# zhengyk19/vit-rpe-rope

Measured on AMD Instinct MI355X. Metric: train images/sec, CIFAR-10 ViT d=192 L=6 H=6, higher is better.
Workload: dtype bf16; 1 GPU; CIFAR-10-shaped 32x32 patch4 ViT d=192 L=6 H=6, --pos_encoding rope-axial theta=100, bf16, full train step (fwd+CE+bwd+AdamW), random-init weights; per_gpu_batch=512, global_batch=512, parallelism=dp1, hip_graph=True

## Files before the change

vit-rpe-rope_amd/csrc/tail2.hip:

```cpp
#include "common.h"
#include <type_traits>
#include <stdlib.h>

#ifndef T2_RB
#define T2_RB 6
#endif
#ifndef T2_NV
#define T2_NV 8
#endif

namespace vitpe {

struct Tail2Args {
  const void* a;
  const void* xin;
  const void* wp;
  const float* bp;
  const float* gamma;
  const float* beta;
  const void* w1;
  const float* b1;
  const void* w2;
  const float* b2;
  void* xmid;
  float* mean2;
  float* rstd2;
  void* xn_out;
  void* gp_out;
  void* h_out;
  void* out;
  float* mean_out;
  float* rstd_out;
  int M, HID;
  float eps2, eps_next;
  unsigned long long* census;
};

constexpr int T2_D = 192, T2_NT = 12, T2_KS = 6, T2_WAVES = 9;
constexpr int T2_THREADS = 64 * (T2_WAVES + 2);
constexpr int T2F_THREADS = 64 * (T2_WAVES + 3);
constexpr int T2_MAXHID = 1536, T2_NFLAG = T2_MAXHID / 64 + 10;
constexpr int T2_CH = 64, T2_CNT = T2_CH / 16, T2_CKS = T2_CH / 32;
constexpr int T2_HALF = T2_CNT * T2_KS;
constexpr int T2_SLABF = 2 * T2_HALF;
static_assert(T2_NT * T2_CKS == T2_HALF, "slab halves");

VITPE_DEV float t2_xg_sum(float v) {
  auto r = __builtin_amdgcn_permlane16_swap(__float_as_uint(v), __float_as_uint(v), false, false);
  v = __uint_as_float(r[0]) + __uint_as_float(r[1]);
  auto q = __builtin_amdgcn_permlane32_swap(__float_as_uint(v), __float_as_uint(v), false, false);
  return __uint_as_float(q[0]) + __uint_as_float(q[1]);
}

#ifndef T2_LOADER_PRIO
#define T2_LOADER_PRIO 3
#endif
#ifndef T2_AUX_HID
#define T2_AUX_HID 2
#endif
#ifndef T2_AUX_ROW
#define T2_AUX_ROW 0
#endif
struct T2Row {
  __amdgpu_buffer_rsrc_t rsrc;
  int off;
  VITPE_DEV T2Row operator+(int elems) const { return T2Row{rsrc, off + 2 * elems}; }
};
VITPE_DEV T2Row t2_row(void* base, int row0, int row, int ld) {
  const __amdgpu_buffer_rsrc_t r = __builtin_amdgcn_make_buffer_rsrc(reinterpret_cast<bf16*>(base) + (size_t)row0 * ld, 0, 0x7fffffff, 0x00020000);
  return T2Row{r, (row - row0) * ld * 2};
}
typedef __attribute__((ext_vector_type(4))) unsigned t2_u32x4;

template <int AUX>
VITPE_DEV void t2_store_pair(const T2Row& row, int nt0, int g, const f32x4& o0, const f32x4& o1) {
  uint32_t lo[2], hi[2];
#pragma unroll
  for (int w2 = 0; w2 < 2; ++w2) {
    bf16x2 pa, pb;
    pa[0] = (bf16)o0[2 * w2]; pa[1] = (bf16)o0[2 * w2 + 1];
    pb[0] = (bf16)o1[2 * w2]; pb[1] = (bf16)o1[2 * w2 + 1];
    const auto r = __builtin_amdgcn_permlane16_swap(__builtin_bit_cast(uint32_t, pa), __builtin_bit_cast(uint32_t, pb), false, false);
    lo[w2] = r[0]; hi[w2] = r[1];
  }
  const int f0 = 16 * (nt0 + (g & 1)) + 8 * (g >> 1);
  __builtin_amdgcn_raw_buffer_store_b128((t2_u32x4){lo[0], lo[1], hi[0], hi[1]}, row.rsrc, row.off + 2 * f0, 0, AUX);
}

template <int AUX>
VITPE_DEV void t2_store_pair_f16(const T2Row& row, int nt0, int g, const f32x4& o0, const f32x4& o1) {
  uint32_t lo[2], hi[2];
#pragma unroll
  for (int w2 = 0; w2 < 2; ++w2) {
    const uint32_t pa = __builtin_bit_cast(uint32_t, __builtin_amdgcn_cvt_pkrtz(o0[2 * w2], o0[2 * w2 + 1]));
    const uint32_t pb = __builtin_bit_cast(uint32_t, __builtin_amdgcn_cvt_pkrtz(o1[2 * w2], o1[2 * w2 + 1]));
    const auto r = __builtin_amdgcn_permlane16_swap(pa, pb, false, false);
    lo[w2] = r[0]; hi[w2] = r[1];
  }
  const int f0 = 16 * (nt0 + (g & 1)) + 8 * (g >> 1);
  __builtin_amdgcn_raw_buffer_store_b128((t2_u32x4){lo[0], lo[1], hi[0], hi[1]}, row.rsrc, row.off + 2 * f0, 0, AUX);
}

template <int AUX>
VITPE_DEV void t2_store_frag(const T2Row& row, int ks, int g, const Frag<bf16>& f) {
  const t2_u32x4 d = __builtin_bit_cast(t2_u32x4, f.v);
  const auto r0 = __builtin_amdgcn_permlane16_swap(d[0], d[2], false, false);
  const auto r1 = __builtin_amdgcn_permlane16_swap(d[1], d[3], false, false);
  const int f0 = 16 * (2 * ks + (g & 1)) + 8 * (g >> 1);
  __builtin_amdgcn_raw_buffer_store_b128((t2_u32x4){r0[0], r1[0], r0[1], r1[1]}, row.rsrc, row.off + 2 * f0, 0, AUX);
}

template <int NTL, int KSL, int R>
VITPE_DEV void t2_gemm_code(const bf16* wb, const Frag<bf16>* bf, f32x4* acc) {
  constexpr int TOT = NTL * KSL;
  static_assert(TOT >= R, "ring deeper than the product");
  Frag<bf16> w[R];
#pragma unroll
  for (int i = 0; i < R - 1; ++i) w[i] = ld_frag(wb + ((i % NTL) * KSL + i / NTL) * 512);
#pragma unroll
  for (int q = 0; q < TOT; ++q) {
    if (q + R - 1 < TOT) {
      const int n = q + R - 1;
      w[n % R] = ld_frag(wb + ((n % NTL) * KSL + n / NTL) * 512);
    }
    mma(w[q % R], bf[q / NTL], acc[q % NTL]);
  }
}
template <int TOT, int R, int NV>
VITPE_DEV void t2_gemm_order() {
  __builtin_amdgcn_sched_group_barrier(0x100, R - 1, 0);
#pragma unroll
  for (int q = 0; q < TOT; ++q) {
    if (q + R - 1 < TOT) __builtin_amdgcn_sched_group_barrier(0x100, 1, 0);
    __builtin_amdgcn_sched_group_barrier(0x008, 1, 0);
    if (NV > 0) __builtin_amdgcn_sched_group_barrier(0x002, NV, 0);
  }
}
template <int NTL, int KSL, int R>
VITPE_DEV void t2_gemm(const bf16* wb, const Frag<bf16>* bf, f32x4* acc) {
  __builtin_amdgcn_sched_barrier(0);
  t2_gemm_code<NTL, KSL, R>(wb, bf, acc);
  t2_gemm_order<NTL * KSL, R, 0>();
  __builtin_amdgcn_sched_barrier(0);
}

VITPE_DEV void t2_gelu(float x, float& h, float& g) {
  constexpr float C = 0.39894228040143267794f;
  const float ax = fabsf(x);
  const float T = __builtin_amdgcn_rcpf(fmaf(ax, 0.3275911f * 0.70710678118654752440f, 1.0f));
  float q = fmaf(T, 1.061405429f / (2.f * C), -1.453152027f / (2.f * C));
  q = fmaf(T, q, 1.421413741f / (2.f * C));
  q = fmaf(T, q, -0.284496736f / (2.f * C));
  q = fmaf(T, q, 0.254829592f / (2.f * C));
  const float E = __builtin_amdgcn_exp2f(fmaf(x * x, -0.72134752044448170368f, -1.32574806473615827f));
  const float H = (q * T) * E;
  h = fmaf(-ax, H, fmaxf(x, 0.f));
  const float r = fmaf(ax, E, -H);
  g = x >= 0.f ? 1.0f + r : -r;
}

template <bool F1, bool F2, int NV, int R = 8, class GFn>
VITPE_DEV void t2_step(const bf16* w1f, const bf16* w2f, const Frag<bf16> (&bf)[T2_KS], f32x4 (&a1n)[2],
                       const Frag<bf16>& hprev, f32x4 (&acc2)[T2_NT], GFn gfn) {
  constexpr int TOT = (F1 ? 12 : 0) + (F2 ? 12 : 0);
  __builtin_amdgcn_sched_barrier(0);
  if (TOT > 0) {
    auto frag_ptr = [&](int q) -> const bf16* {
      const bool is2 = (F1 && F2) ? (q % 2 == 0) : F2;
      const int j = (F1 && F2) ? q / 2 : q;
// ... 307 lines not shown
      }
    }
    stamp(8);

    {
      const T2Row outr = t2_row(a.out, 16 * tile0, rowc, D);
      float s1 = 0.f;
  #pragma unroll
      for (int nt = 0; nt < NT; ++nt) {
        const f32x4 rv = ld4(xmr + 16 * nt + 4 * g);
  #pragma unroll
        for (int r = 0; r < 4; ++r) { acc2[nt][r] = to_f32(from_f32<T>(acc2[nt][r] + rv[r])); s1 += acc2[nt][r]; }
      }
  #pragma unroll
      for (int nt = 0; nt < NT; nt += 2) t2_store_pair<T2_AUX_ROW>(outr, nt, g, acc2[nt], acc2[nt + 1]);
      if (a.mean_out != nullptr) {
        const float mean = t2_xg_sum(s1) * invD;
        float s2 = 0.f;
  #pragma unroll
        for (int nt = 0; nt < NT; ++nt)
  #pragma unroll
          for (int r = 0; r < 4; ++r) { const float d = acc2[nt][r] - mean; s2 += d * d; }
        const float var = t2_xg_sum(s2) * invD;
        if (g == 0) { a.mean_out[rowc] = mean; a.rstd_out[rowc] = 1.0f / sqrtf(var + a.eps_next); }
      }
    }
    stamp(9);
  };
  if (half >= 0) body(std::true_type{});
  else body(std::false_type{});
}

struct Tail2BwdArgs {
  const void* dy;
  const void* gp;
  const void* xmid;
  const float* mean2;
  const float* rstd2;
  const float* gamma;
  const void* w2t;
  const void* w1t;
  const void* wpt;
  void* du;
  void* dxmid;
  void* da;
  float* dgamma;
  float* dbeta;
  int M, HID;
  const void* dqkv;
  const void* wqt;
  const void* x1;
  const float* mean1;
  const float* rstd1;
  const float* gamma1;
  const void* dres1;
  float* dgamma1;
  float* dbeta1;
  int K1;
};

VITPE_DEV void t2_unpack_pair(const Chunk16& v, f32x4& o0, f32x4& o1) {
#pragma unroll
  for (int w2 = 0; w2 < 2; ++w2) {
    const auto r = __builtin_amdgcn_permlane16_swap(v[w2], v[2 + w2], false, false);
    o0[2 * w2] = __uint_as_float(r[0] << 16);
    o0[2 * w2 + 1] = __uint_as_float(r[0] & 0xffff0000u);
    o1[2 * w2] = __uint_as_float(r[1] << 16);
    o1[2 * w2 + 1] = __uint_as_float(r[1] & 0xffff0000u);
  }
}

VITPE_DEV void t2_unpack_pair_f16(const Chunk16& v, f32x4& o0, f32x4& o1) {
#pragma unroll
  for (int w2 = 0; w2 < 2; ++w2) {
    const auto r = __builtin_amdgcn_permlane16_swap(v[w2], v[2 + w2], false, false);
    const uint32_t ra = r[0], rb = r[1];
    o0[2 * w2] = (float)__builtin_bit_cast(_Float16, (unsigned short)(ra & 0xffffu));
    o0[2 * w2 + 1] = (float)__builtin_bit_cast(_Float16, (unsigned short)(ra >> 16));
    o1[2 * w2] = (float)__builtin_bit_cast(_Float16, (unsigned short)(rb & 0xffffu));
    o1[2 * w2 + 1] = (float)__builtin_bit_cast(_Float16, (unsigned short)(rb >> 16));
  }
}

template <int CTRL> VITPE_DEV float t2_dppc(float v) {
  return __builtin_bit_cast(float, __builtin_amdgcn_update_dpp(0, __builtin_bit_cast(int, v), CTRL, 0xf, 0xf, true));
}
VITPE_DEV float t2_colsum8(const float (&t)[8], int c) {
  const bool b3 = (c & 8) != 0, b2 = (c & 4) != 0, b1 = (c & 2) != 0;
  float u[4], w[2];
#pragma unroll
  for (int k = 0; k < 4; ++k) u[k] = (b3 ? t[4 + k] : t[k]) + t2_dppc<0x128>(b3 ? t[k] : t[4 + k]);
#pragma unroll
  for (int k = 0; k < 2; ++k) w[k] = (b2 ? u[2 + k] : u[k]) + t2_dppc<0x141>(b2 ? u[k] : u[2 + k]);
  const float x = (b1 ? w[1] : w[0]) + t2_dppc<0x4E>(b1 ? w[0] : w[1]);
  return x + t2_dppc<0xB1>(x);
}

VITPE_DEV void t2_ln_backward(f32x4 (&acc)[T2_NT], const bf16* xrow, const bf16* rrow, float mean, float rstd,
                              const float* sGam, float* sAcc, int c, int g, float valid, const T2Row& orow) {
  constexpr int D = T2_D, NT = T2_NT;
  bf16x4 xmv[NT];
#pragma unroll
  for (int nt = 0; nt < NT; ++nt) xmv[nt] = *reinterpret_cast<const bf16x4*>(xrow + 16 * nt);
  const float invD = 1.0f / (float)D;
  float s1 = 0.f, s2 = 0.f;
#pragma unroll
  for (int nt = 0; nt < NT; ++nt) {
    __builtin_amdgcn_sched_barrier(0);
    const f32x4 gam = *reinterpret_cast<const f32x4*>(sGam + 16 * nt + 4 * g);
    float tot[8];
#pragma unroll
    for (int r = 0; r < 4; ++r) {
      const float xhat = ((float)xmv[nt][r] - mean) * rstd;
      const float dxn = acc[nt][r];
      tot[r] = dxn * xhat * valid;
      tot[4 + r] = dxn * valid;
      const float gy = dxn * gam[r];
      s1 += gy;
      s2 = fmaf(gy, xhat, s2);
    }
    const float sel = t2_colsum8(tot, c);
    asm volatile("" : "+v"(s1), "+v"(s2));
    if (!(c & 1)) atomicAdd(&sAcc[(c < 8 ? 0 : D - 4) + 16 * nt + 4 * g + (c >> 1)], sel);
  }
  const float m1 = t2_xg_sum(s1) * invD, m2 = t2_xg_sum(s2) * invD;
  bf16x4 rv[NT];
#pragma unroll
  for (int nt = 0; nt < NT; ++nt) rv[nt] = *reinterpret_cast<const bf16x4*>(rrow + 16 * nt);
#pragma unroll
  for (int nt = 0; nt < NT; ++nt) {
    __builtin_amdgcn_sched_barrier(0);
    uint2 xw = __builtin_bit_cast(uint2, xmv[nt]);
    asm volatile("" : "+v"(xw.x), "+v"(xw.y));
    const bf16x4 xb = __builtin_bit_cast(bf16x4, xw);
    const f32x4 gam = *reinterpret_cast<const f32x4*>(sGam + 16 * nt + 4 * g);
#pragma unroll
    for (int r = 0; r < 4; ++r) {
      const float xhat = ((float)xb[r] - mean) * rstd;
      const float gy = acc[nt][r] * gam[r];
      acc[nt][r] = to_f32(from_f32<bf16>(fmaf(rstd, gy - m1 - xhat * m2, (float)rv[nt][r])));
    }
  }
#pragma unroll
  for (int nt = 0; nt < NT; nt += 2) t2_store_pair<T2_AUX_ROW>(orow, nt, g, acc[nt], acc[nt + 1]);
}

VITPE_DEV void t2_flush_colsums(float* sAcc, int* sFin, int nactive, int lane, float* dgamma, float* dbeta) {
  asm volatile("s_waitcnt lgkmcnt(0)" ::: "memory");
  int fin = 0;
  if (lane == 0) fin = atomicAdd(sFin, 1);
  fin = __builtin_amdgcn_readfirstlane(fin);
  if (fin == nactive - 1) {
    for (int i = lane; i < T2_D; i += 64) {
      atomicAdd(dgamma + i, __hip_atomic_load(&sAcc[i], __ATOMIC_RELAXED, __HIP_MEMORY_SCOPE_WORKGROUP));
      atomicAdd(dbeta + i, __hip_atomic_load(&sAcc[T2_D + i], __ATOMIC_RELAXED, __HIP_MEMORY_SCOPE_WORKGROUP));
    }
  }
}

template <bool PRE>
__global__ __launch_bounds__(T2_THREADS) void block_tail2_bwd_kernel(Tail2BwdArgs a) {
  using T = bf16;
  constexpr int D = T2_D, NT = T2_NT, KS = T2_KS;
  __shared__ __attribute__((aligned(16))) T sW[3 * T2_SLABF * 512];
  __shared__ __attribute__((aligned(16))) float sGam[T2_D], sGam1[PRE ? T2_D : 4];
  __shared__ float sAcc[2 * T2_D], sAcc1[PRE ? 2 * T2_D : 4];
  __shared__ int sReady[T2_NFLAG], sDone[T2_NFLAG], sFin;

  const int lane = threadIdx.x & 63, c = lane & 15, g = lane >> 4;
  const int wave = __builtin_amdgcn_readfirstlane(threadIdx.x >> 6);
  const int HID = a.HID, nchunk = HID / T2_CH, nsub = 2 * nchunk;
  const int nkc = PRE ? a.K1 / 64 : 0, Q = (nkc + 1) / 2, QB = nkc / 2;
  const int ntiles = (a.M + 15) / 16, base = ntiles / (int)gridDim.x, rem = ntiles % (int)gridDim.x;
  const int tile0 = (int)blockIdx.x * base + min((int)blockIdx.x, rem), ntile_wg = base + ((int)blockIdx.x < rem ? 1 : 0);
  const bool active = wave < ntile_wg;
  const int row = 16 * (tile0 + wave) + c;
  const int rowc = min(row, a.M - 1);
  const float valid = row < a.M ? 1.0f : 0.0f;

  if (threadIdx.x < T2_NFLAG) { sReady[threadIdx.x] = 0; sDone[threadIdx.x] = 0; }
  if (threadIdx.x == 0) sFin = 0;
  for (int i = threadIdx.x; i < 2 * D; i += T2_THREADS) { sAcc[i] = 0.f; if (PRE) sAcc1[i] = 0.f; }
  for (int i = threadIdx.x; i < D; i += T2_THREADS) { sGam[i] = a.gamma[i]; if (PRE) sGam1[i] = a.gamma1[i]; }

  auto dma1 = [&](const T* src_frag, int dst_frag) {
    __builtin_amdgcn_global_load_lds((const __attribute__((address_space(1))) void*)(src_frag + lane * 8),
                                     (__attribute__((address_space(3))) void*)(sW + dst_frag * 512), 16, 0, 0);
  };
  if (wave >= T2_WAVES) {
    __builtin_amdgcn_s_setprio(T2_LOADER_PRIO);
    const bool is1 = wave == T2_WAVES;
    const int nq = is1 ? Q : QB, njobs = nq + nchunk;
    const int half = is1 ? 0 : T2_HALF;
    auto job_slab = [&](int j) { return j < nq ? j : Q + (j - nq) + (is1 ? 0 : 1); };
    auto dma_job = [&](int j) {
      const T* src;
      if (j < nq) src = reinterpret_cast<const T*>(a.wqt) + ((size_t)j * T2_SLABF + half) * 512;
      else src = (is1 ? reinterpret_cast<const T*>(a.w2t) : reinterpret_cast<const T*>(a.w1t)) + (size_t)(j - nq) * T2_HALF * 512;
      const int b0 = ((job_slab(j) + 2) % 3) * T2_SLABF + half;
#pragma unroll
      for (int f = 0; f < T2_HALF; ++f) dma1(src + (size_t)f * 512, b0 + f);
    };
    auto wait_done = [&](int k) {
      while (__builtin_amdgcn_readfirstlane(__hip_atomic_load(&sDone[k], __ATOMIC_RELAXED, __HIP_MEMORY_SCOPE_WORKGROUP)) < ntile_wg)
        __builtin_amdgcn_s_sleep(2);
      asm volatile("" ::: "memory");
    };
    auto raise = [&](int sl) {
      asm volatile("" ::: "memory");
      if (lane == 0) atomicAdd(&sReady[sl], 1);
    };
    __builtin_amdgcn_s_waitcnt(0x0070);
    asm volatile("s_barrier" ::: "memory");
    int issued = 0, raised = 0;
    auto top_up = [&]() {
      while (issued < njobs && issued - raised < 2) {
        const int g2 = job_slab(issued);
        if (g2 >= 3) {
          if (raised < issued && job_slab(raised) <= g2 - 3) break;
          wait_done(g2 - 2);
        }
        dma_job(issued++);
      }
    };
    top_up();
    while (raised < njobs) {
      if (issued - raised - 1 >= 1) __builtin_amdgcn_s_waitcnt(0x4F78);
      else __builtin_amdgcn_s_waitcnt(0x0F70);
      raise(job_slab(raised));
      ++raised;
      top_up();
    }
    wait_done(Q + nchunk + 1);
#pragma unroll
    for (int f = 0; f < NT * KS / 2; ++f) {
      const int ff = (is1 ? 0 : NT * KS / 2) + f;
      dma1(reinterpret_cast<const T*>(a.wpt) + (size_t)ff * 512, ff);
    }
    __builtin_amdgcn_s_waitcnt(0x0F70);
    raise(Q + nchunk + 1);
    return;
  }
  auto wait_ready = [&](int gs) {
    const int s = gs - Q;
    const int need = gs < Q ? 1 + (2 * gs + 1 < nkc ? 1 : 0) : s > nchunk ? 2 : (s < nchunk ? 1 : 0) + (s >= 1 ? 1 : 0);
    while (__builtin_amdgcn_readfirstlane(__hip_atomic_load(&sReady[gs], __ATOMIC_RELAXED, __HIP_MEMORY_SCOPE_WORKGROUP)) < need)
      __builtin_amdgcn_s_sleep(1);
    asm volatile("" ::: "memory");
  };
  auto signal_done = [&](int k) {
    asm volatile("s_waitcnt lgkmcnt(0)" ::: "memory");
    if (lane == 0) atomicAdd(&sDone[k], 1);
  };
  auto slab_ptr = [&](int gs) { return sW + ((gs + 2) % 3) * T2_SLABF * 512 + lane * 8; };

  Frag<T> bf[KS];
  const T* const dqr = PRE ? reinterpret_cast<const T*>(a.dqkv) + (size_t)rowc * a.K1 + 8 * g : nullptr;
  Frag<T> bqa[4], bqb[4];
  if (active) {
    if (PRE) {
#pragma unroll
      for (int i = 0; i < 4; ++i) bqa[i] = ld_frag(dqr + 32 * min(i, a.K1 / 32 - 1));
    } else {
      const T* dr = reinterpret_cast<const T*>(a.dy) + (size_t)rowc * D + 4 * g;
#pragma unroll
      for (int ks = 0; ks < KS; ++ks) {
        const bf16x4 lo = *reinterpret_cast<const bf16x4*>(dr + 32 * ks), hi = *reinterpret_cast<const bf16x4*>(dr + 32 * ks + 16);
        bf[ks].v = __builtin_shufflevector(lo, hi, 0, 1, 2, 3, 4, 5, 6, 7);
      }
    }
  }
  __builtin_amdgcn_s_waitcnt(0x0070);
  asm volatile("s_barrier" ::: "memory");
  if (!active) return;

  if (PRE) {
    f32x4 acc[NT];
#pragma unroll
    for (int nt = 0; nt < NT; ++nt) acc[nt] = (f32x4){0.f, 0.f, 0.f, 0.f};
    const int nks = a.K1 / 32;
    auto qslab = [&](int q, const Frag<T> (&cur)[4], Frag<T> (&nxt)[4]) {
      if (q + 1 < Q) {
#pragma unroll
        for (int i = 0; i < 4; ++i) nxt[i] = ld_frag(dqr + 32 * min(4 * (q + 1) + i, nks - 1));
      }
      wait_ready(q);
      const T* wb = slab_ptr(q);
      t2_gemm<NT, 2, 8>(wb, cur, acc);
      if (4 * q + 2 < nks) t2_gemm<NT, 2, 8>(wb + T2_HALF * 512, cur + 2, acc);
      signal_done(q + 1);
    };
    for (int q = 0; q < Q; q += 2) {
      qslab(q, bqa, bqb);
      if (q + 1 < Q) qslab(q + 1, bqb, bqa);
    }
    t2_ln_backward(acc, reinterpret_cast<const T*>(a.x1) + (size_t)rowc * D + 4 * g,
                   reinterpret_cast<const T*>(a.dres1) + (size_t)rowc * D + 4 * g, a.mean1[rowc], a.rstd1[rowc], sGam1, sAcc1,
                   c, g, valid, t2_row(const_cast<void*>(a.dy), 16 * tile0, rowc, D));
#pragma unroll
    for (int ks = 0; ks < KS; ++ks) bf[ks] = acc_to_frag<T>(acc[2 * ks], acc[2 * ks + 1]);
  }

  const T* const gpr = reinterpret_cast<const T*>(a.gp) + (size_t)rowc * HID + 16 * (g & 1) + 8 * (g >> 1);
  const T2Row dur = t2_row(a.du, 16 * tile0, rowc, HID);
  Chunk16 gq[2];
#pragma unroll
  for (int t = 0; t < 2; ++t) gq[t] = *reinterpret_cast<const Chunk16*>(gpr + 32 * t);
  f32x4 acc2[NT];
#pragma unroll
  for (int nt = 0; nt < NT; ++nt) acc2[nt] = (f32x4){0.f, 0.f, 0.f, 0.f};
  f32x4 aX[2], aY[2];
  Frag<T> hP, hQ;
  const f32x4 z4 = {0.f, 0.f, 0.f, 0.f};
  auto gstage = [&](const f32x4 (&a1c)[2], Chunk16& slot, int t, Frag<T>& hnew) {
    f32x4 g0, g1, d0, d1;
    t2_unpack_pair_f16(slot, g0, g1);
    if (t + 2 < nsub) slot = *reinterpret_cast<const Chunk16*>(gpr + 32 * (t + 2));
#pragma unroll
    for (int r = 0; r < 4; ++r) { d0[r] = a1c[0][r] * g0[r]; d1[r] = a1c[1][r] * g1[r]; }
    t2_store_pair<T2_AUX_HID>(dur + 32 * t, 0, g, d0, d1);
    hnew = acc_to_frag<T>(d0, d1);
  };
  constexpr int NVB = 3, RB = T2_RB;

  wait_ready(Q);
  {
    const T* wb = slab_ptr(Q);
    aX[0] = z4; aX[1] = z4;
    t2_step<true, false, 0, RB>(wb, wb, bf, aX, hQ, acc2, [&]() {});
    aY[0] = z4; aY[1] = z4;
    t2_step<true, false, 2 * NVB, RB>(wb + 2 * KS * 512, wb, bf, aY, hQ, acc2, [&]() { gstage(aX, gq[0], 0, hP); });
    signal_done(Q + 1);
  }
  for (int p = 1; p < nchunk; ++p) {
    wait_ready(Q + p);
    const T* wb = slab_ptr(Q + p);
    const T* w2b = wb + T2_HALF * 512;
    aX[0] = z4; aX[1] = z4;
    t2_step<true, true, NVB, RB>(wb, w2b, bf, aX, hP, acc2, [&]() { gstage(aY, gq[1], 2 * p - 1, hQ); });
    aY[0] = z4; aY[1] = z4;
    t2_step<true, true, NVB, RB>(wb + 2 * KS * 512, w2b + NT * 512, bf, aY, hQ, acc2, [&]() { gstage(aX, gq[0], 2 * p, hP); });
    signal_done(Q + p + 1);
  }
  wait_ready(Q + nchunk);
  {
    const T* w2b = slab_ptr(Q + nchunk) + T2_HALF * 512;
    const int tl = nsub - 1;
    t2_step<false, true, 2 * NVB, RB>(w2b, w2b, bf, aX, hP, acc2, [&]() { gstage(aY, gq[1], tl, hQ); });
    t2_step<false, true, 0, RB>(w2b, w2b + NT * 512, bf, aX, hQ, acc2, [&]() {});
    signal_done(Q + nchunk + 1);
  }
  t2_ln_backward(acc2, reinterpret_cast<const T*>(a.xmid) + (size_t)rowc * D + 4 * g,
                 reinterpret_cast<const T*>(a.dy) + (size_t)rowc * D + 4 * g, a.mean2[rowc], a.rstd2[rowc], sGam, sAcc, c, g,
                 valid, t2_row(a.dxmid, 16 * tile0, rowc, D));
#pragma unroll
  for (int ks = 0; ks < KS; ++ks) bf[ks] = acc_to_frag<T>(acc2[2 * ks], acc2[2 * ks + 1]);
  f32x4 accA[NT];
#pragma unroll
  for (int nt = 0; nt < NT; ++nt) accA[nt] = z4;
  wait_ready(Q + nchunk + 1);
  t2_gemm<NT, KS, 12>(sW + lane * 8, bf, accA);
  {
    const T2Row dar = t2_row(a.da, 16 * tile0, rowc, D);
#pragma unroll
    for (int nt = 0; nt < NT; nt += 2) t2_store_pair<T2_AUX_ROW>(dar, nt, g, accA[nt], accA[nt + 1]);
  }
  asm volatile("s_waitcnt lgkmcnt(0)" ::: "memory");
  int fin = 0;
  if (lane == 0) fin = atomicAdd(&sFin, 1);
  fin = __builtin_amdgcn_readfirstlane(fin);
  if (fin == ntile_wg - 1) {
    for (int i = lane; i < D; i += 64) {
      atomicAdd(a.dgamma + i, __hip_atomic_load(&sAcc[i], __ATOMIC_RELAXED, __HIP_MEMORY_SCOPE_WORKGROUP));
      atomicAdd(a.dbeta + i, __hip_atomic_load(&sAcc[D + i], __ATOMIC_RELAXED, __HIP_MEMORY_SCOPE_WORKGROUP));
      if (PRE) {
        atomicAdd(a.dgamma1 + i, __hip_atomic_load(&sAcc1[i], __ATOMIC_RELAXED, __HIP_MEMORY_SCOPE_WORKGROUP));
        atomicAdd(a.dbeta1 + i, __hip_atomic_load(&sAcc1[D + i], __ATOMIC_RELAXED, __HIP_MEMORY_SCOPE_WORKGROUP));
      }
    }
  }
}

struct LnBwd2Args {
  const void* dy;
  const void* wt;
  const void* x;
  const float* mean;
  const float* rstd;
  const float* gamma;
  const void* dres;
  void* dx;
  float* dgamma;
  float* dbeta;
  int M, K;
};

__global__ __launch_bounds__(T2_THREADS) void ln_bwd2_kernel(LnBwd2Args a) {
  using T = bf16;
  constexpr int D = T2_D, NT = T2_NT, KS = T2_KS, SLF = NT * KS;
  __shared__ __attribute__((aligned(16))) T sW[2 * SLF * 512];
  __shared__ __attribute__((aligned(16))) float sGam[T2_D];
  __shared__ float sAcc[2 * T2_D];
  __shared__ int sReady[T2_NFLAG], sDone[T2_NFLAG], sFin;

  const int lane = threadIdx.x & 63, c = lane & 15, g = lane >> 4;
  const int wave = __builtin_amdgcn_readfirstlane(threadIdx.x >> 6);
  const int K = a.K, nslab = K / D;
  const int ntiles = (a.M + 15) / 16, base = ntiles / (int)gridDim.x, rem = ntiles % (int)gridDim.x;
  const int tile0 = (int)blockIdx.x * base + min((int)blockIdx.x, rem), ntile_wg = base + ((int)blockIdx.x < rem ? 1 : 0);
  const bool active = wave < ntile_wg;
  const int row = 16 * (tile0 + wave) + c;
  const int rowc = min(row, a.M - 1);
  const float valid = row < a.M ? 1.0f : 0.0f;

  if (threadIdx.x < T2_NFLAG) { sReady[threadIdx.x] = 0; sDone[threadIdx.x] = 0; }
  if (threadIdx.x == 0) sFin = 0;
  for (int i = threadIdx.x; i < 2 * D; i += T2_THREADS) sAcc[i] = 0.f;
  for (int i = threadIdx.x; i < D; i += T2_THREADS) sGam[i] = a.gamma[i];

  if (wave >= T2_WAVES) {
    __builtin_amdgcn_s_setprio(T2_LOADER_PRIO);
    const int half = wave == T2_WAVES ? 0 : SLF / 2;
    auto dma_half = [&](int sl) {
#pragma unroll
      for (int f = 0; f < SLF / 2; ++f) {
        const T* src = reinterpret_cast<const T*>(a.wt) + ((size_t)sl * SLF + half + f) * 512 + lane * 8;
        __builtin_amdgcn_global_load_lds((const __attribute__((address_space(1))) void*)src,
                                         (__attribute__((address_space(3))) void*)(sW + ((sl & 1) * SLF + half + f) * 512), 16, 0, 0);
      }
    };
    __builtin_amdgcn_s_waitcnt(0x0070);
    asm volatile("s_barrier" ::: "memory");
    dma_half(0);
    if (nslab > 1) dma_half(1);
    for (int sl = 0; sl < nslab; ++sl) {
      if (sl + 1 < nslab) asm volatile("s_waitcnt vmcnt(36)" ::: "memory");
      else __builtin_amdgcn_s_waitcnt(0x0F70);
      asm volatile("" ::: "memory");
      if (lane == 0) atomicAdd(&sReady[sl], 1);
      if (sl + 2 < nslab) {
        while (__builtin_amdgcn_readfirstlane(__hip_atomic_load(&sDone[sl], __ATOMIC_RELAXED, __HIP_MEMORY_SCOPE_WORKGROUP)) < ntile_wg)
          __builtin_amdgcn_s_sleep(2);
        asm volatile("" ::: "memory");
        dma_half(sl + 2);
      }
    }
    return;
  }
  __builtin_amdgcn_s_waitcnt(0x0070);
  asm volatile("s_barrier" ::: "memory");
  if (!active) return;

  const T* const dr = reinterpret_cast<const T*>(a.dy) + (size_t)rowc * K + 8 * g;
  Frag<T> bfa[KS], bfb[KS];
#pragma unroll
  for (int ks = 0; ks < KS; ++ks) bfa[ks] = ld_frag(dr + 32 * ks);
  f32x4 acc[NT];
#pragma unroll
  for (int nt = 0; nt < NT; ++nt) acc[nt] = (f32x4){0.f, 0.f, 0.f, 0.f};
  auto chunk = [&](int sl, const Frag<T> (&cur)[KS], Frag<T> (&nxt)[KS]) {
    if (sl + 1 < nslab) {
#pragma unroll
      for (int ks = 0; ks < KS; ++ks) nxt[ks] = ld_frag(dr + (sl + 1) * D + 32 * ks);
    }
    while (__builtin_amdgcn_readfirstlane(__hip_atomic_load(&sReady[sl], __ATOMIC_RELAXED, __HIP_MEMORY_SCOPE_WORKGROUP)) < 2)
      __builtin_amdgcn_s_sleep(1);
    asm volatile("" ::: "memory");
    {
      const T* wb = sW + (sl & 1) * SLF * 512 + lane * 8;
#pragma unroll
      for (int kcl = 0; kcl < 3; ++kcl) t2_gemm<NT, 2, 8>(wb + kcl * T2_HALF * 512, cur + 2 * kcl, acc);
    }
    asm volatile("s_waitcnt lgkmcnt(0)" ::: "memory");
    if (lane == 0) atomicAdd(&sDone[sl], 1);
  };
  for (int sl = 0; sl < nslab; sl += 2) {
    chunk(sl, bfa, bfb);
    if (sl + 1 < nslab) chunk(sl + 1, bfb, bfa);
  }
  t2_ln_backward(acc, reinterpret_cast<const T*>(a.x) + (size_t)rowc * D + 4 * g,
                 reinterpret_cast<const T*>(a.dres) + (size_t)rowc * D + 4 * g, a.mean[rowc], a.rstd[rowc], sGam, sAcc, c, g,
                 valid, t2_row(a.dx, 16 * tile0, rowc, D));
  t2_flush_colsums(sAcc, &sFin, ntile_wg, lane, a.dgamma, a.dbeta);
}

template <typename T>
__global__ void pack_frags_kernel(const float* __restrict__ w, T* __restrict__ dst, int R, int Cc, int kchunk, int phi) {
  const long long total = (long long)R * Cc;
  const int NTr = R / 16, KSC = kchunk / 32;
  for (long long idx = (long long)blockIdx.x * blockDim.x + threadIdx.x; idx < total; idx += (long long)gridDim.x * blockDim.x) {
    const int e = (int)(idx & 7), l = (int)((idx >> 3) & 63);
    long long blk = idx >> 9;
    const int ks = (int)(blk % KSC); blk /= KSC;
    const int nt = (int)(blk % NTr);
    const int kc = (int)(blk / NTr);
    const int cc = l & 15, g = l >> 4;
    const int k = phi ? (e < 4 ? 4 * g + e : 16 + 4 * g + e - 4) : 8 * g + e;
    dst[idx] = from_f32<T>(w[(size_t)(16 * nt + cc) * Cc + (size_t)kchunk * kc + 32 * ks + k]);
  }
}

}

using namespace vitpe;

extern "C" int vitpe_pack_weight_frags(int dtype, const float* w, void* packed, int R, int C, int kchunk, int phi,
                                       hipStream_t stream) {
  VITPE_REQUIRE(w && packed && R > 0 && C > 0 && kchunk > 0 && R % 16 == 0 && kchunk % 32 == 0 && C % kchunk == 0 &&
                (dtype == 0 || dtype == 1));
  const long long total = (long long)R * C;
  const unsigned blocks = (unsigned)min((total + 255) / 256, (long long)2048);
  if (dtype == 1) hipLaunchKernelGGL(pack_frags_kernel<bf16>, dim3(blocks), dim3(256), 0, stream, w, (bf16*)packed, R, C, kchunk, phi);
  else hipLaunchKernelGGL(pack_frags_kernel<float>, dim3(blocks), dim3(256), 0, stream, w, (float*)packed, R, C, kchunk, phi);
  VITPE_CHECK_LAUNCH();
}

extern "C" int vitpe_block_tail2_supported(int dtype, int D, int HID) {
  return dtype == 1 && D == T2_D && HID >= 2 * T2_CH && HID % T2_CH == 0 && HID <= T2_MAXHID;
}

static int tail2_launch(int dtype, const void* attn_out, const void* x_in, const void* Wp_packed, const float* bp,
                        const float* gamma, const float* beta, void* x_mid, float* mean2, float* rstd2,
                        void* xn_out, const void* W1_packed, const float* b1, const void* W2_packed,
                        const float* b2, void* gp_out, void* h_out, void* out, float* mean_out, float* rstd_out,
                        float eps2, float eps_next, int M, int D, int HID, unsigned long long* census, hipStream_t stream) {
  VITPE_REQUIRE(attn_out && x_in && Wp_packed && bp && gamma && beta && x_mid && mean2 && rstd2 && W1_packed && b1 &&
                W2_packed && b2 && out && M >= 0);
  VITPE_REQUIRE((mean_out == nullptr) == (rstd_out == nullptr) && (gp_out == nullptr) == (h_out == nullptr));
  if (!vitpe_block_tail2_supported(dtype, D, HID)) return (int)hipErrorNotSupported;
  if (M == 0) return 0;
  Tail2Args a{};
  a.a = attn_out; a.xin = x_in; a.wp = Wp_packed; a.bp = bp; a.gamma = gamma; a.beta = beta; a.w1 = W1_packed; a.b1 = b1;
  a.w2 = W2_packed; a.b2 = b2; a.xmid = x_mid; a.mean2 = mean2; a.rstd2 = rstd2; a.xn_out = xn_out; a.gp_out = gp_out;
  a.h_out = h_out; a.out = out; a.mean_out = mean_out; a.rstd_out = rstd_out; a.M = M; a.HID = HID; a.eps2 = eps2;
  a.eps_next = eps_next;
  const int ntiles = (M + 15) / 16;
  int grid;
  if (ntiles <= 256 * 8) grid = (ntiles + 7) / 8;
  else grid = 256 * ((ntiles + 256 * T2_WAVES - 1) / (256 * T2_WAVES));
  a.census = census;
  if (census != nullptr) {
    VITPE_REQUIRE(gp_out != nullptr);
    hipLaunchKernelGGL((block_tail2_fwd_kernel<true, true>), dim3(grid), dim3(T2F_THREADS), 0, stream, a);
  } else if (gp_out != nullptr) {
    hipLaunchKernelGGL((block_tail2_fwd_kernel<true, false>), dim3(grid), dim3(T2F_THREADS), 0, stream, a);
  } else {
    hipLaunchKernelGGL((block_tail2_fwd_kernel<false, false>), dim3(grid), dim3(T2F_THREADS), 0, stream, a);
  }
  VITPE_CHECK_LAUNCH();
}

extern "C" int vitpe_block_tail2_fwd(int dtype, const void* attn_out, const void* x_in, const void* Wp_packed, const float* bp,
                                     const float* gamma, const float* beta, void* x_mid, float* mean2, float* rstd2,
                                     void* xn_out, const void* W1_packed, const float* b1, const void* W2_packed,
                                     const float* b2, void* gp_out, void* h_out, void* out, float* mean_out, float* rstd_out,
                                     float eps2, float eps_next, int M, int D, int HID, hipStream_t stream) {
  return tail2_launch(dtype, attn_out, x_in, Wp_packed, bp, gamma, beta, x_mid, mean2, rstd2, xn_out, W1_packed, b1, W2_packed,
                      b2, gp_out, h_out, out, mean_out, rstd_out, eps2, eps_next, M, D, HID, nullptr, stream);
}

extern "C" int vitpe_debug_tail2_census(const void* attn_out, const void* x_in, const void* Wp_packed, const float* bp,
                                        const float* gamma, const float* beta, void* x_mid, float* mean2, float* rstd2,
                                        void* xn_out, const void* W1_packed, const float* b1, const void* W2_packed,
                                        const float* b2, void* gp_out, void* h_out, void* out, float* mean_out,
                                        float* rstd_out, int M, int HID, unsigned long long* census, hipStream_t stream) {
// ... 64 lines not shown
```

Baseline: 364,000 images/sec.

## Load row pairs as full cache-line chunks and redistribute via DPP/permlane swaps

Global loads of activations and gradients (dy, dqkv, x, residual, gp) and the du stores in the fused tail backward kernels are restructured. Each lane pair now reads or writes full 16-byte chunks spanning two adjacent rows, instead of scattered 8-byte or 16-byte pieces per row. The data is then exchanged between lanes with DPP row swaps and permlane16 swaps to rebuild the MFMA fragment layout. This aims to coalesce memory accesses into whole cache lines, at the cost of extra cross-lane shuffle instructions and more register pressure from keeping the even-stage du results live.

```diff
diff --git a/vit-rpe-rope_amd/csrc/tail2.hip b/vit-rpe-rope_amd/csrc/tail2.hip
--- a/vit-rpe-rope_amd/csrc/tail2.hip
+++ b/vit-rpe-rope_amd/csrc/tail2.hip
@@ -72,8 +72,7 @@
 }
 typedef __attribute__((ext_vector_type(4))) unsigned t2_u32x4;
 
-template <int AUX>
-VITPE_DEV void t2_store_pair(const T2Row& row, int nt0, int g, const f32x4& o0, const f32x4& o1) {
+VITPE_DEV t2_u32x4 t2_pack_pair(const f32x4& o0, const f32x4& o1) {
   uint32_t lo[2], hi[2];
 #pragma unroll
   for (int w2 = 0; w2 < 2; ++w2) {
@@ -83,8 +82,28 @@
     const auto r = __builtin_amdgcn_permlane16_swap(__builtin_bit_cast(uint32_t, pa), __builtin_bit_cast(uint32_t, pb), false, false);
     lo[w2] = r[0]; hi[w2] = r[1];
   }
+  return (t2_u32x4){lo[0], lo[1], hi[0], hi[1]};
+}
+template <int AUX>
+VITPE_DEV void t2_store_pair(const T2Row& row, int nt0, int g, const f32x4& o0, const f32x4& o1) {
   const int f0 = 16 * (nt0 + (g & 1)) + 8 * (g >> 1);
-  __builtin_amdgcn_raw_buffer_store_b128((t2_u32x4){lo[0], lo[1], hi[0], hi[1]}, row.rsrc, row.off + 2 * f0, 0, AUX);
+  __builtin_amdgcn_raw_buffer_store_b128(t2_pack_pair(o0, o1), row.rsrc, row.off + 2 * f0, 0, AUX);
+}
+
+VITPE_DEV void t2_line_xchg(bool even, const t2_u32x4& a, const t2_u32x4& b, t2_u32x4& o0, t2_u32x4& o1) {
+#pragma unroll
+  for (int w = 0; w < 4; ++w) {
+    const uint32_t na = (uint32_t)__builtin_amdgcn_update_dpp(0, (int)a[w], 0xB1, 0xf, 0xf, true);
+    const uint32_t nb = (uint32_t)__builtin_amdgcn_update_dpp(0, (int)b[w], 0xB1, 0xf, 0xf, true);
+    o0[w] = even ? a[w] : nb;
+    o1[w] = even ? na : b[w];
+  }
+}
+VITPE_DEV void t2_lines_to_frags(bool even, Frag<bf16>& f0, Frag<bf16>& f1) {
+  t2_u32x4 o0, o1;
+  t2_line_xchg(even, __builtin_bit_cast(t2_u32x4, f0.v), __builtin_bit_cast(t2_u32x4, f1.v), o0, o1);
+  f0.v = __builtin_bit_cast(bf16x8, o0);
+  f1.v = __builtin_bit_cast(bf16x8, o1);
 }
 
 template <int AUX>
@@ -558,6 +577,27 @@
   }
 }
 
+VITPE_DEV void t2_load_rows(bool even, const bf16* line, int step, bf16x4 (&v)[T2_NT]) {
+  Chunk16 l[6];
+#pragma unroll
+  for (int m = 0; m < 3; ++m) {
+    l[2 * m] = *reinterpret_cast<const Chunk16*>(line + 64 * m);
+    l[2 * m + 1] = *reinterpret_cast<const Chunk16*>(line + step + 64 * m);
+  }
+#pragma unroll
+  for (int m = 0; m < 3; ++m) {
+    Chunk16 h[2];
+    t2_line_xchg(even, l[2 * m], l[2 * m + 1], h[0], h[1]);
+#pragma unroll
+    for (int s = 0; s < 2; ++s) {
+      const auto r0 = __builtin_amdgcn_permlane16_swap(h[s][0], h[s][2], false, false);
+      const auto r1 = __builtin_amdgcn_permlane16_swap(h[s][1], h[s][3], false, false);
+      v[4 * m + 2 * s] = __builtin_bit_cast(bf16x4, (uint2){r0[0], r1[0]});
+      v[4 * m + 2 * s + 1] = __builtin_bit_cast(bf16x4, (uint2){r0[1], r1[1]});
+    }
+  }
+}
+
 template <int CTRL> VITPE_DEV float t2_dppc(float v) {
   return __builtin_bit_cast(float, __builtin_amdgcn_update_dpp(0, __builtin_bit_cast(int, v), CTRL, 0xf, 0xf, true));
 }
@@ -572,12 +612,12 @@
   return x + t2_dppc<0xB1>(x);
 }
 
-VITPE_DEV void t2_ln_backward(f32x4 (&acc)[T2_NT], const bf16* xrow, const bf16* rrow, float mean, float rstd,
+VITPE_DEV void t2_ln_backward(f32x4 (&acc)[T2_NT], const bf16* xline, const bf16* rline, int lstep, float mean, float rstd,
                               const float* sGam, float* sAcc, int c, int g, float valid, const T2Row& orow) {
   constexpr int D = T2_D, NT = T2_NT;
+  const bool even = (c & 1) == 0;
   bf16x4 xmv[NT];
-#pragma unroll
-  for (int nt = 0; nt < NT; ++nt) xmv[nt] = *reinterpret_cast<const bf16x4*>(xrow + 16 * nt);
+  t2_load_rows(even, xline, lstep, xmv);
   const float invD = 1.0f / (float)D;
   float s1 = 0.f, s2 = 0.f;
 #pragma unroll
@@ -601,8 +641,7 @@
   }
   const float m1 = t2_xg_sum(s1) * invD, m2 = t2_xg_sum(s2) * invD;
   bf16x4 rv[NT];
-#pragma unroll
-  for (int nt = 0; nt < NT; ++nt) rv[nt] = *reinterpret_cast<const bf16x4*>(rrow + 16 * nt);
+  t2_load_rows(even, rline, lstep, rv);
 #pragma unroll
   for (int nt = 0; nt < NT; ++nt) {
     __builtin_amdgcn_sched_barrier(0);
@@ -731,19 +770,25 @@
   auto slab_ptr = [&](int gs) { return sW + ((gs + 2) % 3) * T2_SLABF * 512 + lane * 8; };
 
   Frag<T> bf[KS];
-  const T* const dqr = PRE ? reinterpret_cast<const T*>(a.dqkv) + (size_t)rowc * a.K1 + 8 * g : nullptr;
+  const bool even = (c & 1) == 0;
+  const int lrow = min(row & ~1, a.M - 1), lnext = min((row & ~1) + 1, a.M - 1) - lrow;
+  const T* const dql = PRE ? reinterpret_cast<const T*>(a.dqkv) + (size_t)lrow * a.K1 + 32 * (c & 1) + 8 * g : nullptr;
+  const int dqstep = PRE ? lnext * a.K1 : 0;
+  const int lpiece = 32 * (c & 1) + 16 * (g & 1) + 8 * (g >> 1);
+  const size_t lrowD = (size_t)lrow * D + lpiece;
   Frag<T> bqa[4], bqb[4];
+  auto ld_qlines = [&](Frag<T> (&f)[4], int q) {
+#pragma unroll
+    for (int i = 0; i < 4; ++i) f[i] = ld_frag(dql + (i & 1) * dqstep + 64 * min(2 * q + (i >> 1), nkc - 1));
+  };
   if (active) {
     if (PRE) {
-#pragma unroll
-      for (int i = 0; i < 4; ++i) bqa[i] = ld_frag(dqr + 32 * min(i, a.K1 / 32 - 1));
+      ld_qlines(bqa, 0);
     } else {
-      const T* dr = reinterpret_cast<const T*>(a.dy) + (size_t)rowc * D + 4 * g;
-#pragma unroll
-      for (int ks = 0; ks < KS; ++ks) {
-        const bf16x4 lo = *reinterpret_cast<const bf16x4*>(dr + 32 * ks), hi = *reinterpret_cast<const bf16x4*>(dr + 32 * ks + 16);
-        bf[ks].v = __builtin_shufflevector(lo, hi, 0, 1, 2, 3, 4, 5, 6, 7);
-      }
+      bf16x4 dv[NT];
+      t2_load_rows(even, reinterpret_cast<const T*>(a.dy) + lrowD, lnext * D, dv);
+#pragma unroll
+      for (int ks = 0; ks < KS; ++ks) bf[ks].v = __builtin_shufflevector(dv[2 * ks], dv[2 * ks + 1], 0, 1, 2, 3, 4, 5, 6, 7);
     }
   }
   __builtin_amdgcn_s_waitcnt(0x0070);
@@ -755,11 +800,10 @@
 #pragma unroll
     for (int nt = 0; nt < NT; ++nt) acc[nt] = (f32x4){0.f, 0.f, 0.f, 0.f};
     const int nks = a.K1 / 32;
-    auto qslab = [&](int q, const Frag<T> (&cur)[4], Frag<T> (&nxt)[4]) {
-      if (q + 1 < Q) {
-#pragma unroll
-        for (int i = 0; i < 4; ++i) nxt[i] = ld_frag(dqr + 32 * min(4 * (q + 1) + i, nks - 1));
-      }
+    auto qslab = [&](int q, Frag<T> (&cur)[4], Frag<T> (&nxt)[4]) {
+      if (q + 1 < Q) ld_qlines(nxt, q + 1);
+      t2_lines_to_frags(even, cur[0], cur[1]);
+      t2_lines_to_frags(even, cur[2], cur[3]);
       wait_ready(q);
       const T* wb = slab_ptr(q);
       t2_gemm<NT, 2, 8>(wb, cur, acc);
@@ -770,31 +814,50 @@
       qslab(q, bqa, bqb);
       if (q + 1 < Q) qslab(q + 1, bqb, bqa);
     }
-    t2_ln_backward(acc, reinterpret_cast<const T*>(a.x1) + (size_t)rowc * D + 4 * g,
-                   reinterpret_cast<const T*>(a.dres1) + (size_t)rowc * D + 4 * g, a.mean1[rowc], a.rstd1[rowc], sGam1, sAcc1,
-                   c, g, valid, t2_row(const_cast<void*>(a.dy), 16 * tile0, rowc, D));
+    t2_ln_backward(acc, reinterpret_cast<const T*>(a.x1) + lrowD, reinterpret_cast<const T*>(a.dres1) + lrowD, lnext * D,
+                   a.mean1[rowc], a.rstd1[rowc], sGam1, sAcc1, c, g, valid, t2_row(const_cast<void*>(a.dy), 16 * tile0, rowc, D));
 #pragma unroll
     for (int ks = 0; ks < KS; ++ks) bf[ks] = acc_to_frag<T>(acc[2 * ks], acc[2 * ks + 1]);
   }
 
-  const T* const gpr = reinterpret_cast<const T*>(a.gp) + (size_t)rowc * HID + 16 * (g & 1) + 8 * (g >> 1);
-  const T2Row dur = t2_row(a.du, 16 * tile0, rowc, HID);
+  const int lstep = lnext * HID;
+  const T* const gpl = reinterpret_cast<const T*>(a.gp) + (size_t)lrow * HID + lpiece;
+  const T2Row dul = t2_row(a.du, 16 * tile0, lrow, HID) + lpiece;
   Chunk16 gq[2];
-#pragma unroll
-  for (int t = 0; t < 2; ++t) gq[t] = *reinterpret_cast<const Chunk16*>(gpr + 32 * t);
+  gq[0] = *reinterpret_cast<const Chunk16*>(gpl);
+  gq[1] = *reinterpret_cast<const Chunk16*>(gpl + lstep);
+  Chunk16 godd;
+  t2_u32x4 duh;
   f32x4 acc2[NT];
 #pragma unroll
   for (int nt = 0; nt < NT; ++nt) acc2[nt] = (f32x4){0.f, 0.f, 0.f, 0.f};
   f32x4 aX[2], aY[2];
   Frag<T> hP, hQ;
   const f32x4 z4 = {0.f, 0.f, 0.f, 0.f};
-  auto gstage = [&](const f32x4 (&a1c)[2], Chunk16& slot, int t, Frag<T>& hnew) {
+  auto gstage_even = [&](const f32x4 (&a1c)[2], int p, Frag<T>& hnew) {
     f32x4 g0, g1, d0, d1;
-    t2_unpack_pair_f16(slot, g0, g1);
-    if (t + 2 < nsub) slot = *reinterpret_cast<const Chunk16*>(gpr + 32 * (t + 2));
+    Chunk16 cur;
+    t2_line_xchg(even, gq[0], gq[1], cur, godd);
+    if (p + 1 < nchunk) {
+      gq[0] = *reinterpret_cast<const Chunk16*>(gpl + 64 * (p + 1));
+      gq[1] = *reinterpret_cast<const Chunk16*>(gpl + lstep + 64 * (p + 1));
+    }
+    t2_unpack_pair_f16(cur, g0, g1);
 #pragma unroll
     for (int r = 0; r < 4; ++r) { d0[r] = a1c[0][r] * g0[r]; d1[r] = a1c[1][r] * g1[r]; }
-    t2_store_pair<T2_AUX_HID>(dur + 32 * t, 0, g, d0, d1);
+    duh = t2_pack_pair(d0, d1);
+    asm volatile("" : "+v"(duh));
+    hnew = acc_to_frag<T>(d0, d1);
+  };
+  auto gstage_odd = [&](const f32x4 (&a1c)[2], int p, Frag<T>& hnew) {
+    f32x4 g0, g1, d0, d1;
+    t2_unpack_pair_f16(godd, g0, g1);
+#pragma unroll
+    for (int r = 0; r < 4; ++r) { d0[r] = a1c[0][r] * g0[r]; d1[r] = a1c[1][r] * g1[r]; }
+    t2_u32x4 l0, l1;
+    t2_line_xchg(even, duh, t2_pack_pair(d0, d1), l0, l1);
+    __builtin_amdgcn_raw_buffer_store_b128(l0, dul.rsrc, dul.off + 128 * p, 0, T2_AUX_HID);
+    __builtin_amdgcn_raw_buffer_store_b128(l1, dul.rsrc, dul.off + 2 * lstep + 128 * p, 0, T2_AUX_HID);
     hnew = acc_to_frag<T>(d0, d1);
   };
   constexpr int NVB = 3, RB = T2_RB;
@@ -805,7 +868,7 @@
     aX[0] = z4; aX[1] = z4;
     t2_step<true, false, 0, RB>(wb, wb, bf, aX, hQ, acc2, [&]() {});
     aY[0] = z4; aY[1] = z4;
-    t2_step<true, false, 2 * NVB, RB>(wb + 2 * KS * 512, wb, bf, aY, hQ, acc2, [&]() { gstage(aX, gq[0], 0, hP); });
+    t2_step<true, false, 2 * NVB, RB>(wb + 2 * KS * 512, wb, bf, aY, hQ, acc2, [&]() { gstage_even(aX, 0, hP); });
     signal_done(Q + 1);
   }
   for (int p = 1; p < nchunk; ++p) {
@@ -813,22 +876,20 @@
     const T* wb = slab_ptr(Q + p);
     const T* w2b = wb + T2_HALF * 512;
     aX[0] = z4; aX[1] = z4;
-    t2_step<true, true, NVB, RB>(wb, w2b, bf, aX, hP, acc2, [&]() { gstage(aY, gq[1], 2 * p - 1, hQ); });
+    t2_step<true, true, NVB, RB>(wb, w2b, bf, aX, hP, acc2, [&]() { gstage_odd(aY, p - 1, hQ); });
     aY[0] = z4; aY[1] = z4;
-    t2_step<true, true, NVB, RB>(wb + 2 * KS * 512, w2b + NT * 512, bf, aY, hQ, acc2, [&]() { gstage(aX, gq[0], 2 * p, hP); });
+    t2_step<true, true, NVB, RB>(wb + 2 * KS * 512, w2b + NT * 512, bf, aY, hQ, acc2, [&]() { gstage_even(aX, p, hP); });
     signal_done(Q + p + 1);
   }
   wait_ready(Q + nchunk);
   {
     const T* w2b = slab_ptr(Q + nchunk) + T2_HALF * 512;
-    const int tl = nsub - 1;
-    t2_step<false, true, 2 * NVB, RB>(w2b, w2b, bf, aX, hP, acc2, [&]() { gstage(aY, gq[1], tl, hQ); });
+    t2_step<false, true, 2 * NVB, RB>(w2b, w2b, bf, aX, hP, acc2, [&]() { gstage_odd(aY, nchunk - 1, hQ); });
     t2_step<false, true, 0, RB>(w2b, w2b + NT * 512, bf, aX, hQ, acc2, [&]() {});
     signal_done(Q + nchunk + 1);
   }
-  t2_ln_backward(acc2, reinterpret_cast<const T*>(a.xmid) + (size_t)rowc * D + 4 * g,
-                 reinterpret_cast<const T*>(a.dy) + (size_t)rowc * D + 4 * g, a.mean2[rowc], a.rstd2[rowc], sGam, sAcc, c, g,
-                 valid, t2_row(a.dxmid, 16 * tile0, rowc, D));
+  t2_ln_backward(acc2, reinterpret_cast<const T*>(a.xmid) + lrowD, reinterpret_cast<const T*>(a.dy) + lrowD, lnext * D,
+                 a.mean2[rowc], a.rstd2[rowc], sGam, sAcc, c, g, valid, t2_row(a.dxmid, 16 * tile0, rowc, D));
 #pragma unroll
   for (int ks = 0; ks < KS; ++ks) bf[ks] = acc_to_frag<T>(acc2[2 * ks], acc2[2 * ks + 1]);
   f32x4 accA[NT];
@@ -927,18 +988,22 @@
   asm volatile("s_barrier" ::: "memory");
   if (!active) return;
 
-  const T* const dr = reinterpret_cast<const T*>(a.dy) + (size_t)rowc * K + 8 * g;
+  const bool even = (c & 1) == 0;
+  const int lrow = min(row & ~1, a.M - 1), lnext = min((row & ~1) + 1, a.M - 1) - lrow, dstep = lnext * K;
+  const T* const dl = reinterpret_cast<const T*>(a.dy) + (size_t)lrow * K + 32 * (c & 1) + 8 * g;
   Frag<T> bfa[KS], bfb[KS];
-#pragma unroll
-  for (int ks = 0; ks < KS; ++ks) bfa[ks] = ld_frag(dr + 32 * ks);
+  auto ld_lines = [&](Frag<T> (&f)[KS], int sl) {
+#pragma unroll
+    for (int ks = 0; ks < KS; ++ks) f[ks] = ld_frag(dl + (ks & 1) * dstep + sl * D + 64 * (ks >> 1));
+  };
+  ld_lines(bfa, 0);
   f32x4 acc[NT];
 #pragma unroll
   for (int nt = 0; nt < NT; ++nt) acc[nt] = (f32x4){0.f, 0.f, 0.f, 0.f};
-  auto chunk = [&](int sl, const Frag<T> (&cur)[KS], Frag<T> (&nxt)[KS]) {
-    if (sl + 1 < nslab) {
-#pragma unroll
-      for (int ks = 0; ks < KS; ++ks) nxt[ks] = ld_frag(dr + (sl + 1) * D + 32 * ks);
-    }
+  auto chunk = [&](int sl, Frag<T> (&cur)[KS], Frag<T> (&nxt)[KS]) {
+    if (sl + 1 < nslab) ld_lines(nxt, sl + 1);
+#pragma unroll
+    for (int ks = 0; ks < KS; ks += 2) t2_lines_to_frags(even, cur[ks], cur[ks + 1]);
     while (__builtin_amdgcn_readfirstlane(__hip_atomic_load(&sReady[sl], __ATOMIC_RELAXED, __HIP_MEMORY_SCOPE_WORKGROUP)) < 2)
       __builtin_amdgcn_s_sleep(1);
     asm volatile("" ::: "memory");
@@ -954,9 +1019,9 @@
     chunk(sl, bfa, bfb);
     if (sl + 1 < nslab) chunk(sl + 1, bfb, bfa);
   }
-  t2_ln_backward(acc, reinterpret_cast<const T*>(a.x) + (size_t)rowc * D + 4 * g,
-                 reinterpret_cast<const T*>(a.dres) + (size_t)rowc * D + 4 * g, a.mean[rowc], a.rstd[rowc], sGam, sAcc, c, g,
-                 valid, t2_row(a.dx, 16 * tile0, rowc, D));
+  const size_t lrowD = (size_t)lrow * D + 32 * (c & 1) + 16 * (g & 1) + 8 * (g >> 1);
+  t2_ln_backward(acc, reinterpret_cast<const T*>(a.x) + lrowD, reinterpret_cast<const T*>(a.dres) + lrowD, lnext * D,
+                 a.mean[rowc], a.rstd[rowc], sGam, sAcc, c, g, valid, t2_row(a.dx, 16 * tile0, rowc, D));
   t2_flush_colsums(sAcc, &sFin, ntile_wg, lane, a.dgamma, a.dbeta);
 }
 
```

After: 374,500 images/sec (median of 6 runs). +2.9%, better.
